# phd3/presto-1

Hardware: AMD Instinct MI355X
Metric: probe_rows_per_sec (higher is better)
Workload: dtype int64+f64

## Files before the change

### presto-1_amd/csrc/basic.hip

```cpp
#include "kernels.h"
#include "device_hash.h"

namespace tgpu {
namespace k {

constexpr int kBlock = 256;
constexpr int kWaves = kBlock / 64;

constexpr int kScanItems = 8;
constexpr int kScanTile = kBlock * kScanItems;

template <typename T> __device__ __forceinline__ T wave_inclusive_scan(T v)
{
    const int lane = threadIdx.x & 63;
#pragma unroll
    for (int d = 1; d < 64; d <<= 1) {
        T t = __shfl_up(v, d, 64);
        if (lane >= d) v += t;
    }
    return v;
}

template <typename T> __device__ __forceinline__ T block_exclusive_scan(T v, T *total, T *lds )
{
    const int lane = threadIdx.x & 63, wave = threadIdx.x >> 6;
    T inc = wave_inclusive_scan(v);
    if (lane == 63) lds[wave] = inc;
    __syncthreads();
    if (threadIdx.x == 0) {
        T run = 0;
#pragma unroll
        for (int w = 0; w < kWaves; w++) { T t = lds[w]; lds[w] = run; run += t; }
        lds[kWaves] = run;
    }
    __syncthreads();
    T prefix = lds[wave] + inc - v;
    *total = lds[kWaves];
    __syncthreads();
    return prefix;
}

__device__ __forceinline__ void scan_load8(const int32_t *__restrict__ in, int64_t idx, int64_t n, bool aligned, int32_t v[kScanItems])
{
    if (aligned && idx + kScanItems <= n) {
        const int4 a = *reinterpret_cast<const int4 *>(in + idx), b = *reinterpret_cast<const int4 *>(in + idx + 4);
        v[0] = a.x; v[1] = a.y; v[2] = a.z; v[3] = a.w; v[4] = b.x; v[5] = b.y; v[6] = b.z; v[7] = b.w;
        return;
    }
#pragma unroll
    for (int i = 0; i < kScanItems; i++) v[i] = idx + i < n ? in[idx + i] : 0;
}

constexpr int kScanMaxBlocks = 2048;

__global__ void __launch_bounds__(kBlock) scan_range_sums_i32(const int32_t *__restrict__ in, int64_t n, int64_t range, int64_t *__restrict__ range_sums)
{
    __shared__ int64_t lds[kWaves + 1];
    const bool aligned = (reinterpret_cast<uintptr_t>(in) & 15) == 0;
    const int64_t a = (int64_t)blockIdx.x * range, z = a + range < n ? a + range : n;
    int64_t s = 0;
    for (int64_t base = a; base < z; base += kScanTile) {
        int32_t v[kScanItems];
        scan_load8(in, base + (int64_t)threadIdx.x * kScanItems, z, aligned, v);
#pragma unroll
        for (int i = 0; i < kScanItems; i++) s += v[i];
    }
    int64_t total;
    block_exclusive_scan<int64_t>(s, &total, lds);
    if (threadIdx.x == 0) range_sums[blockIdx.x] = total;
}

__global__ void __launch_bounds__(kBlock) scan_ranges_i32(const int32_t *__restrict__ in, int32_t *__restrict__ out, int64_t n, int64_t range,
                                                           const int64_t *__restrict__ range_prefix)
{
    __shared__ int64_t lds[kWaves + 1];
    const bool aligned = (reinterpret_cast<uintptr_t>(in) & 15) == 0, out_aligned = (reinterpret_cast<uintptr_t>(out) & 15) == 0;
    const int64_t a = (int64_t)blockIdx.x * range, z = a + range < n ? a + range : n;
    int64_t carry = range_prefix[blockIdx.x];
    for (int64_t base = a; base < z; base += kScanTile) {
        const int64_t idx = base + (int64_t)threadIdx.x * kScanItems;
        int32_t v[kScanItems];
        scan_load8(in, idx, z, aligned, v);
        int64_t s = 0;
#pragma unroll
        for (int i = 0; i < kScanItems; i++) s += v[i];
        int64_t total;
        int64_t prefix = carry + block_exclusive_scan<int64_t>(s, &total, lds);
        int32_t o[kScanItems];
#pragma unroll
        for (int i = 0; i < kScanItems; i++) {
            o[i] = (int32_t)prefix;
            prefix += v[i];
        }
        if (out_aligned && idx + kScanItems <= z) {
            *reinterpret_cast<int4 *>(out + idx) = make_int4(o[0], o[1], o[2], o[3]);
            *reinterpret_cast<int4 *>(out + idx + 4) = make_int4(o[4], o[5], o[6], o[7]);
        } else {
#pragma unroll
            for (int i = 0; i < kScanItems; i++)
                if (idx + i < z) out[idx + i] = o[i];
        }
        carry += total;
    }
}

__global__ void __launch_bounds__(kBlock) scan_small_i64(const int64_t *__restrict__ in, int64_t *__restrict__ out, int64_t n, int64_t *total_out)
{
    __shared__ int64_t lds[kWaves + 1];
    int64_t carry = 0;
    for (int64_t base = 0; base < n; base += kBlock) {
        int64_t idx = base + threadIdx.x;
        int64_t v = idx < n ? in[idx] : 0;
        int64_t total;
        int64_t p = block_exclusive_scan<int64_t>(v, &total, lds);
        if (idx < n) out[idx] = carry + p;
        carry += total;
    }
    if (threadIdx.x == 0 && total_out) *total_out = carry;
}

__global__ void __launch_bounds__(kBlock) scan_one_tile_i32(const int32_t *__restrict__ in, int32_t *__restrict__ out, int64_t n, int64_t *total_out)
{
    __shared__ int64_t lds[kWaves + 1];
    const int64_t base = (int64_t)threadIdx.x * kScanItems;
    int32_t v[kScanItems];
    int64_t s = 0;
#pragma unroll
    for (int i = 0; i < kScanItems; i++) {
        v[i] = base + i < n ? in[base + i] : 0;
        s += v[i];
    }
    int64_t total;
    int64_t prefix = block_exclusive_scan<int64_t>(s, &total, lds);
#pragma unroll
    for (int i = 0; i < kScanItems; i++) {
        if (base + i < n) out[base + i] = (int32_t)prefix;
        prefix += v[i];
    }
    if (threadIdx.x == 0 && total_out) *total_out = total;
}

void exclusive_scan_i32(Context *ctx, const int32_t *in, int32_t *out, int64_t n, int64_t *total_dev)
{
    if (n <= 0) {
        if (total_dev) HIP_CHECK(hipMemsetAsync(total_dev, 0, 8, ctx->stream()));
        return;
    }
    if (n <= kScanTile) {
        scan_one_tile_i32<<<1, kBlock, 0, ctx->stream()>>>(in, out, n, total_dev);
        check_launch("exclusive_scan_i32");
        return;
    }
    const int64_t tiles = ceil_div(n, kScanTile);
    const int64_t tiles_per_range = ceil_div(tiles, (int64_t)kScanMaxBlocks), range = tiles_per_range * kScanTile, ranges = ceil_div(n, range);
    BufferPtr sums = ctx->alloc((size_t)ranges * 8);
    BufferPtr prefix = ctx->alloc((size_t)ranges * 8);
    scan_range_sums_i32<<<(int)ranges, kBlock, 0, ctx->stream()>>>(in, n, range, sums->as<int64_t>());
    scan_small_i64<<<1, kBlock, 0, ctx->stream()>>>(sums->as<int64_t>(), prefix->as<int64_t>(), ranges, total_dev);
    scan_ranges_i32<<<(int)ranges, kBlock, 0, ctx->stream()>>>(in, out, n, range, prefix->as<int64_t>());
    check_launch("exclusive_scan_i32");
}

__global__ void __launch_bounds__(kBlock) hash_rows_kernel(KeyCols keys, int64_t n, int64_t *__restrict__ out)
{
    for (int64_t r = (int64_t)blockIdx.x * kBlock + threadIdx.x; r < n; r += (int64_t)gridDim.x * kBlock) {
        out[r] = tg_hash_row_u(keys, r);
    }
}

void hash_rows(Context *ctx, const KeyCols &keys, int64_t n, int64_t *out)
{
    if (n <= 0) return;
    ProfileScope ps(ctx, "hash_rows");
    hash_rows_kernel<<<grid_for(ctx, n), kBlock, 0, ctx->stream()>>>(keys, n, out);
    check_launch("hash_rows");
}

__global__ void __launch_bounds__(kBlock) any_null_kernel(KeyCols keys, int64_t n, uint8_t *__restrict__ out)
{
    for (int64_t r = (int64_t)blockIdx.x * kBlock + threadIdx.x; r < n; r += (int64_t)gridDim.x * kBlock) {
        uint8_t f = 0;
#pragma unroll
        for (int c = 0; c < TG_MAX_KEY_CHANNELS; c++) {
            if (c >= keys.n) break;
            f |= (keys.c[c].nulls && keys.c[c].nulls[r]) ? 1 : 0;
        }
        out[r] = f;
    }
}

void any_null(Context *ctx, const KeyCols &keys, int64_t n, uint8_t *out)
{
    if (n <= 0) return;
    any_null_kernel<<<grid_for(ctx, n), kBlock, 0, ctx->stream()>>>(keys, n, out);
    check_launch("any_null");
}

template <typename T> __global__ void __launch_bounds__(kBlock) fill_kernel(T *p, T v, int64_t n)
{
    for (int64_t i = (int64_t)blockIdx.x * kBlock + threadIdx.x; i < n; i += (int64_t)gridDim.x * kBlock) p[i] = v;
}
__global__ void __launch_bounds__(kBlock) iota_kernel(int32_t *p, int64_t n)
{
    for (int64_t i = (int64_t)blockIdx.x * kBlock + threadIdx.x; i < n; i += (int64_t)gridDim.x * kBlock) p[i] = (int32_t)i;
}
__global__ void __launch_bounds__(kBlock) widen_kernel(const int32_t *in, int64_t *out, int64_t n)
{
    for (int64_t i = (int64_t)blockIdx.x * kBlock + threadIdx.x; i < n; i += (int64_t)gridDim.x * kBlock) out[i] = in[i];
}

void fill_i32(Context *ctx, int32_t *p, int32_t v, int64_t n)
{
    if (n <= 0) return;
    fill_kernel<int32_t><<<grid_for(ctx, n), kBlock, 0, ctx->stream()>>>(p, v, n);
    check_launch("fill_i32");
}
void fill_u64(Context *ctx, uint64_t *p, uint64_t v, int64_t n)
{
    if (n <= 0) return;
    fill_kernel<uint64_t><<<grid_for(ctx, n), kBlock, 0, ctx->stream()>>>(p, v, n);
    check_launch("fill_u64");
}
void iota_i32(Context *ctx, int32_t *p, int64_t n)
{
    if (n <= 0) return;
    iota_kernel<<<grid_for(ctx, n), kBlock, 0, ctx->stream()>>>(p, n);
    check_launch("iota_i32");
}
void widen_i32_to_i64(Context *ctx, const int32_t *in, int64_t *out, int64_t n)
{
    if (n <= 0) return;
    widen_kernel<<<grid_for(ctx, n), kBlock, 0, ctx->stream()>>>(in, out, n);
    check_launch("widen");
}

__global__ void __launch_bounds__(kBlock) compact_positions_kernel(const int32_t *__restrict__ flags, const int32_t *__restrict__ rank, int64_t n, int32_t *__restrict__ out)
{
    for (int64_t i = (int64_t)blockIdx.x * kBlock + threadIdx.x; i < n; i += (int64_t)gridDim.x * kBlock)
        if (flags[i]) out[rank[i]] = (int32_t)i;
}
void compact_positions(Context *ctx, const int32_t *flags, const int32_t *rank, int64_t n, int32_t *out)
{
    if (n <= 0) return;
    compact_positions_kernel<<<grid_for(ctx, n), kBlock, 0, ctx->stream()>>>(flags, rank, n, out);
}

template <typename T>
__global__ void __launch_bounds__(kBlock) gather_fixed_kernel(const T *__restrict__ src, const uint8_t *__restrict__ src_nulls,
                                                               const int32_t *__restrict__ pos, int64_t n_out,
                                                               T *__restrict__ out, uint8_t *__restrict__ out_nulls)
{
    for (int64_t i = (int64_t)blockIdx.x * kBlock + threadIdx.x; i < n_out; i += (int64_t)gridDim.x * kBlock) {
        int32_t p = pos[i];
        T v = T(0);
        uint8_t isnull = 1;
        if (p >= 0) {
            isnull = src_nulls ? src_nulls[p] : 0;
            v = src[p];
        }
        out[i] = v;
        if (out_nulls) out_nulls[i] = isnull;
    }
}

__global__ void __launch_bounds__(kBlock) gather_len_kernel(const int32_t *__restrict__ offsets, const int32_t *__restrict__ pos,
                                                             int64_t n_out, int32_t *__restrict__ len)
{
    for (int64_t i = (int64_t)blockIdx.x * kBlock + threadIdx.x; i < n_out; i += (int64_t)gridDim.x * kBlock) {
        int32_t p = pos[i];
        len[i] = p >= 0 ? offsets[p + 1] - offsets[p] : 0;
    }
}

__global__ void __launch_bounds__(kBlock) gather_bytes_kernel(const uint8_t *__restrict__ pool, const int32_t *__restrict__ offsets,
                                                               const uint8_t *__restrict__ src_nulls, const int32_t *__restrict__ pos,
                                                               int64_t n_out, const int32_t *__restrict__ out_offsets,
                                                               const int64_t *__restrict__ total, int32_t *__restrict__ out_offsets_end,
                                                               uint8_t *__restrict__ out_pool, uint8_t *__restrict__ out_nulls)
{
    for (int64_t i = (int64_t)blockIdx.x * kBlock + threadIdx.x; i < n_out; i += (int64_t)gridDim.x * kBlock) {
        int32_t p = pos[i];
        uint8_t isnull = 1;
        if (p >= 0) {
            isnull = src_nulls ? src_nulls[p] : 0;
            int32_t a = offsets[p], b = offsets[p + 1], o = out_offsets[i];
            for (int32_t k = a; k < b; k++) out_pool[o + (k - a)] = pool[k];
        }
        if (out_nulls) out_nulls[i] = isnull;
        if (i == n_out - 1) *out_offsets_end = (int32_t)(*total);
    }
}

DeviceColumn gather_column(Context *ctx, const DeviceColumn &src, const int32_t *positions, int64_t n_out, bool negative_is_null)
{
    DeviceColumn out;
    out.type = src.type;
    out.n = n_out;
    const bool need_nulls = src.nulls != nullptr || negative_is_null;
    if (need_nulls) {
        out.nulls_buf = ctx->alloc((size_t)(n_out > 0 ? n_out : 1));
        out.nulls = out.nulls_buf->as<uint8_t>();
    }
// ... 88 lines not shown
```

### presto-1_amd/csrc/join.hip

```cpp
#include "join.h"
#include "kernels.h"
#include "device_hash.h"
#include "device_join.h"

#include <rocprim/rocprim.hpp>

#include <algorithm>
#include <cstdlib>

namespace tgpu {

namespace {

constexpr int kBlock = 256;

using Slot16 = TgSlot16;

__device__ __forceinline__ bool rows_equal_nonnull(const KeyCols &a, int64_t ra, const KeyCols &b, int64_t rb)
{
#pragma unroll
    for (int c = 0; c < TG_MAX_KEY_CHANNELS; c++) {
        if (c >= a.n) break;
        const ColView &x = a.c[c], &y = b.c[c];
        switch (x.type) {
// ... 123 lines not shown
        if (!row_has_null(keys, r)) {
            const int64_t h = hashes[r];
            uint64_t pos = tg_fmix64((uint64_t)h) & mask;
            for (uint64_t iter = 0; iter <= mask; iter++) {
                int *hp = heads + pos * stride;
                int cur = __hip_atomic_load(hp, __ATOMIC_RELAXED, __HIP_MEMORY_SCOPE_AGENT);
                if (cur == -1) {
                    int old = atomicCAS(hp, -1, (int)r);
                    if (old == -1) { slot = (int32_t)pos; break; }
                    cur = old;
                }
                if (tags[cur] == (uint8_t)h && rows_equal_nonnull(keys, cur, keys, r)) {
                    atomicMax(hp, (int)r);
                    slot = (int32_t)pos;
                    dup = true;
                    break;
                }
                pos = (pos + 1) & mask;
                if (iter == mask) atomicExch(&counters[1], 1ull);
            }
        }
        row_slot[r] = slot;
        unsigned long long b = __ballot(dup);
        if (dup && (threadIdx.x & 63) == (__ffsll((long long)b) - 1)) atomicAdd(&counters[0], (unsigned long long)__popcll(b));
    }
}

constexpr long long kUnwrittenKey = (long long)0x8000000000000001ull;
constexpr int kBuildRows = 4;

__device__ __forceinline__ int build_insert_row(const ColView &key, long long k, int r, Slot16 *slots, uint64_t mask, uint64_t pos, long long ks, int head, bool &dup,
                                                unsigned long long *counters)
{
    for (uint64_t iter = 0; iter <= mask; iter++) {
        if (head == -1) {
            const int old = atomicCAS(&slots[pos].head, -1, r);
            if (old == -1) {
                __hip_atomic_store(&slots[pos].key, k, __ATOMIC_RELAXED, __HIP_MEMORY_SCOPE_AGENT);
                return (int)pos;
            }
            head = old;
            ks = __hip_atomic_load(&slots[pos].key, __ATOMIC_RELAXED, __HIP_MEMORY_SCOPE_AGENT);
        }
        const bool same = ks == kUnwrittenKey ? int_key_at(key, head) == k : ks == k;
        if (same) {
            (void)__hip_atomic_fetch_max(&slots[pos].head, r, __ATOMIC_RELAXED, __HIP_MEMORY_SCOPE_AGENT);
            dup = true;
            return (int)pos;
        }
        pos = (pos + 1) & mask;
        const ulonglong2 v = *(const ulonglong2 *)&slots[pos];
        ks = (long long)v.x;
        head = (int)(unsigned int)v.y;
    }
    atomicExch(&counters[1], 1ull);
    return -1;
}

__global__ void __launch_bounds__(kBlock) build_insert_int_kernel(ColView key, int64_t n, Slot16 *slots, uint64_t mask, int32_t *__restrict__ row_slot,
                                                                   unsigned long long *counters, long long *minmax)
{
    long long lo = 0x7fffffffffffffffLL, hi = -0x7fffffffffffffffLL - 1;
    unsigned int my_dups = 0;
    for (int64_t base = (int64_t)blockIdx.x * (kBlock * kBuildRows); base < n; base += (int64_t)gridDim.x * (kBlock * kBuildRows)) {
        long long k[kBuildRows];
        bool live[kBuildRows], claimed[kBuildRows];
        uint64_t pos[kBuildRows];
        ulonglong2 snap[kBuildRows];
        int old[kBuildRows];
#pragma unroll
        for (int u = 0; u < kBuildRows; u++) {
            const int64_t r = base + u * kBlock + threadIdx.x;
            live[u] = r < n && !(key.nulls && key.nulls[r]);
            k[u] = live[u] ? int_key_at(key, r) : 0;
            if (live[u]) {
                lo = k[u] < lo ? k[u] : lo;
                hi = k[u] > hi ? k[u] : hi;
            }
        }
#pragma unroll
        for (int u = 0; u < kBuildRows; u++) {
            pos[u] = tg_slot_of(k[u], mask);
            snap[u] = *(const ulonglong2 *)&slots[live[u] ? pos[u] : 0];
        }
#pragma unroll
        for (int u = 0; u < kBuildRows; u++) {
            claimed[u] = live[u] && (int)(unsigned int)snap[u].y == -1;
            old[u] = 0;
            if (claimed[u]) old[u] = atomicCAS(&slots[pos[u]].head, -1, (int)(base + u * kBlock + threadIdx.x));
        }
#pragma unroll
        for (int u = 0; u < kBuildRows; u++)
            if (claimed[u] && old[u] == -1) __hip_atomic_store(&slots[pos[u]].key, k[u], __ATOMIC_RELAXED, __HIP_MEMORY_SCOPE_AGENT);
#pragma unroll
        for (int u = 0; u < kBuildRows; u++) {
            const int64_t r = base + u * kBlock + threadIdx.x;
            int32_t slot = -1;
            bool dup = false;
            if (claimed[u] && old[u] == -1) slot = (int32_t)pos[u];
            else if (live[u]) {
                long long ks = (long long)snap[u].x;
                int head = (int)(unsigned int)snap[u].y;
                if (claimed[u]) {
                    head = old[u];
                    ks = __hip_atomic_load(&slots[pos[u]].key, __ATOMIC_RELAXED, __HIP_MEMORY_SCOPE_AGENT);
                }
                slot = build_insert_row(key, k[u], (int)r, slots, mask, pos[u], ks, head, dup, counters);
            }
            if (r < n) row_slot[r] = slot;
            my_dups += dup ? 1u : 0u;
        }
    }
    __shared__ unsigned int s_dups[kBlock / 64];
#pragma unroll
    for (int d = 32; d >= 1; d >>= 1) my_dups += __shfl_down(my_dups, d, 64);
    if ((threadIdx.x & 63) == 0) s_dups[threadIdx.x >> 6] = my_dups;
    __syncthreads();
    if (threadIdx.x == 0) {
        unsigned long long total = 0;
#pragma unroll
        for (int w = 0; w < kBlock / 64; w++) total += s_dups[w];
        if (total) atomicAdd(&counters[0], total);
    }
    block_minmax(lo, hi, minmax);
}

__global__ void __launch_bounds__(kBlock) sort_keys_kernel(const int32_t *__restrict__ row_slot, int64_t n, unsigned long long *__restrict__ keys)
{
    for (int64_t r = (int64_t)blockIdx.x * kBlock + threadIdx.x; r < n; r += (int64_t)gridDim.x * kBlock) {
        int32_t s = row_slot[r];
        keys[r] = s < 0 ? ~0ull : (((unsigned long long)(uint32_t)s << 32) | (unsigned long long)(uint32_t)r);
    }
}

__global__ void __launch_bounds__(kBlock) links_kernel(const unsigned long long *__restrict__ sorted, int64_t n, int32_t *__restrict__ links, Slot16 *slots)
{
    for (int64_t i = (int64_t)blockIdx.x * kBlock + threadIdx.x; i < n; i += (int64_t)gridDim.x * kBlock) {
        unsigned long long k = sorted[i];
        if (k == ~0ull) continue;
        int32_t link = -1;
        if (i > 0) {
            unsigned long long p = sorted[i - 1];
            if ((p >> 32) == (k >> 32)) link = (int32_t)(uint32_t)p;
        }
        links[(uint32_t)k] = link;
        if (slots && (i + 1 == n || (sorted[i + 1] >> 32) != (k >> 32))) {
            int64_t first = i;
            while (first > 0 && (sorted[first - 1] >> 32) == (k >> 32)) first--;
            slots[k >> 32].count = (int)(i - first + 1);
        }
    }
}

__global__ void __launch_bounds__(kBlock) key_range_kernel(ColView key, int64_t n, long long *minmax)
{
    long long lo = 0x7fffffffffffffffLL, hi = -0x7fffffffffffffffLL - 1;
    bool descent = false;
    const int64_t stride = (int64_t)gridDim.x * kBlock;
    const int lane = threadIdx.x & 63;
    for (int64_t r0 = (int64_t)blockIdx.x * kBlock + threadIdx.x; r0 < n; r0 += 4 * stride) {
        long long k[4], before[4];
        bool live[4];
#pragma unroll
        for (int u = 0; u < 4; u++) {
            const int64_t r = r0 + u * stride;
            live[u] = r < n;
            const int64_t rc = live[u] ? r : r0;
            live[u] = live[u] && !(key.nulls && key.nulls[rc]);
            k[u] = int_key_at(key, rc);
            before[u] = (lane == 0 && r < n && r > 0) ? int_key_at(key, r - 1) : (-0x7fffffffffffffffLL - 1);
        }
#pragma unroll
        for (int u = 0; u < 4; u++) {
            const int64_t r = r0 + u * stride;
            lo = (live[u] && k[u] < lo) ? k[u] : lo;
            hi = (live[u] && k[u] > hi) ? k[u] : hi;
            const long long up = __shfl_up(k[u], 1, 64);
            const long long pred = lane == 0 ? before[u] : up;
            descent = descent || (r < n && r > 0 && pred >= k[u]);
        }
    }
    block_minmax(lo, hi, minmax);
    if (__any(descent) && (threadIdx.x & 63) == 0) minmax[2] = 1;
}

__global__ void __launch_bounds__(kBlock) build_direct_kernel(ColView key, int64_t n, long long key_min, unsigned long long *bitmap,
                                                               unsigned long long *counters)
{
    const int lane = threadIdx.x & 63;
    unsigned int my_dups = 0;
    for (int64_t base = (int64_t)blockIdx.x * kBlock; base < n; base += (int64_t)gridDim.x * kBlock) {
        const int64_t r = base + threadIdx.x;
        const bool active = r < n && !(key.nulls && key.nulls[r]);
        unsigned long long d = 0;
        if (active) {
            d = (unsigned long long)int_key_at(key, r) - (unsigned long long)key_min;
        }
        const unsigned int word = active ? (unsigned int)(d >> 6) : 0xffffffffu;
        unsigned long long bits = active ? (1ULL << (d & 63)) : 0ULL;
        unsigned int rows = active ? 1u : 0u;
        const unsigned int word_prev = __shfl_up(word, 1, 64);
        const bool head = lane == 0 || word_prev != word;
        const unsigned long long heads = __ballot(head);
        const int run = __popcll(heads & ((2ULL << lane) - 1ULL));
#pragma unroll
        for (int k = 1; k < 64; k <<= 1) {
            const unsigned long long b2 = __shfl_down(bits, k, 64);
            const unsigned int c2 = __shfl_down(rows, k, 64);
            const int run2 = __shfl_down(run, k, 64);
            if (lane + k < 64 && run2 == run) {
                bits |= b2;
                rows += c2;
            }
        }
        if (head && active) {
            const unsigned long long old = atomicOr(&bitmap[word], bits);
            my_dups += (unsigned int)__popcll(old & bits) + (rows - (unsigned int)__popcll(bits));
        }
    }
    __shared__ unsigned int s_dups[kBlock / 64];
#pragma unroll
    for (int d = 32; d >= 1; d >>= 1) my_dups += __shfl_down(my_dups, d, 64);
    if (lane == 0) s_dups[threadIdx.x >> 6] = my_dups;
    __syncthreads();
    if (threadIdx.x == 0) {
        unsigned long long total = 0;
#pragma unroll
        for (int w = 0; w < kBlock / 64; w++) total += s_dups[w];
        if (total) atomicAdd(&counters[0], total);
    }
}

__global__ void __launch_bounds__(kBlock) init_slots_kernel(Slot16 *__restrict__ slots, int64_t capacity)
{
    for (int64_t i = (int64_t)blockIdx.x * kBlock + threadIdx.x; i < capacity; i += (int64_t)gridDim.x * kBlock) {
        Slot16 s;
        s.key = kUnwrittenKey;
        s.head = -1;
        s.count = 1;
        slots[i] = s;
    }
}

__global__ void __launch_bounds__(kBlock) bitmap_popcount_kernel(const unsigned long long *__restrict__ bitmap, int64_t words, int32_t *__restrict__ counts)
{
    for (int64_t i = (int64_t)blockIdx.x * kBlock + threadIdx.x; i < words; i += (int64_t)gridDim.x * kBlock) counts[i] = (int32_t)__popcll(bitmap[i]);
}

__global__ void __launch_bounds__(kBlock) build_rank_kernel(ColView key, int64_t n, long long key_min, const unsigned long long *__restrict__ bitmap,
                                                             const int32_t *__restrict__ rank_base, int32_t *__restrict__ direct)
{
    for (int64_t r = (int64_t)blockIdx.x * kBlock + threadIdx.x; r < n; r += (int64_t)gridDim.x * kBlock) {
        if (key.nulls && key.nulls[r]) continue;
        const unsigned long long d = (unsigned long long)int_key_at(key, r) - (unsigned long long)key_min;
        direct[rank_base[d >> 6] + __popcll(bitmap[d >> 6] & ((1ULL << (d & 63)) - 1ULL))] = (int32_t)r;
    }
}

__global__ void __launch_bounds__(kBlock) bitmap_build_kernel(const int32_t *__restrict__ row_slot, int64_t n, ColView key, long long key_min,
                                                               unsigned long long *bitmap)
{
    for (int64_t r = (int64_t)blockIdx.x * kBlock + threadIdx.x; r < n; r += (int64_t)gridDim.x * kBlock) {
        if (row_slot[r] < 0) continue;
        const unsigned long long d = (unsigned long long)(int_key_at(key, r) - key_min);
        atomicOr(&bitmap[d >> 6], 1ULL << (d & 63));
    }
}

__global__ void __launch_bounds__(kBlock) bloom_build_kernel(const int32_t *__restrict__ row_slot, int64_t n, ColView key, unsigned long long *bloom,
                                                              unsigned long long word_mask)
{
    for (int64_t r = (int64_t)blockIdx.x * kBlock + threadIdx.x; r < n; r += (int64_t)gridDim.x * kBlock) {
        if (row_slot[r] < 0) continue;
        const unsigned long long m = tg_fmix64((unsigned long long)tg_hash_long(int_key_at(key, r)));
        atomicOr(&bloom[tg_bloom_word(m, word_mask)], tg_bloom_mask(m));
    }
}

struct ProbeTable {
    const int *heads;
    const Slot16 *slots;
    const uint8_t *tags;
    const int32_t *links;
    uint64_t mask;
    TgPrefilter pf;
};

template <bool FAST>
__device__ __forceinline__ int find_head(const ProbeTable &t, const KeyCols &build, const KeyCols &probe, int64_t r, int64_t h)
{
    if (FAST) return tg_find_head_int(t.slots, t.mask, t.pf, int_key_at(probe.c[0], r));
    uint64_t pos = tg_fmix64((uint64_t)h) & t.mask;
    for (uint64_t iter = 0; iter <= t.mask; iter++) {
        const int b = t.heads[pos];
        if (b < 0) return -1;
        if (t.tags[b] == (uint8_t)h && rows_equal_nonnull(build, b, probe, r)) return b;
        pos = (pos + 1) & t.mask;
    }
    return -1;
}

template <bool FAST>
__global__ void __launch_bounds__(kBlock) probe_count_kernel(ProbeTable t, KeyCols build, KeyCols probe, const int64_t *__restrict__ hashes, int64_t n,
                                                              int probe_outer, int32_t *__restrict__ heads_out, int32_t *__restrict__ counts)
{
    for (int64_t r = (int64_t)blockIdx.x * kBlock + threadIdx.x; r < n; r += (int64_t)gridDim.x * kBlock) {
        int head = -1, chain = 0;
        if (!row_has_null(probe, r)) {
            if (FAST) head = tg_find_head_int(t.slots, t.mask, t.pf, int_key_at(probe.c[0], r), &chain);
            else head = find_head<FAST>(t, build, probe, r, hashes[r]);
        }
        int32_t c = 0;
        if (head >= 0) {
            c = 1;
            if (t.links) {
                if (FAST && !t.pf.rank_base) c = chain;
                else
                    for (int p = t.links[head]; p >= 0; p = t.links[p]) c++;
            }
        }
        else if (probe_outer) c = 1;
        heads_out[r] = head;
        counts[r] = c;
    }
}

__global__ void __launch_bounds__(kBlock) probe_write_kernel(const int32_t *__restrict__ links, const int32_t *__restrict__ heads, const int32_t *__restrict__ offsets,
                                                              const int32_t *__restrict__ counts, int64_t n, int probe_outer, int32_t *__restrict__ out_probe,
                                                              int32_t *__restrict__ out_build)
{
    for (int64_t r = (int64_t)blockIdx.x * kBlock + threadIdx.x; r < n; r += (int64_t)gridDim.x * kBlock) {
        int head = heads[r];
        int64_t o = offsets[r];
        if (head >= 0) {
            int p = head;
            for (int32_t left = counts[r]; left > 0; left--) {
                out_probe[o] = (int32_t)r;
                out_build[o] = p;
                o++;
                if (left > 1) p = links[p];
            }
        }
        else if (probe_outer) {
            out_probe[o] = (int32_t)r;
            out_build[o] = -1;
        }
    }
}

}

PagesIndexGpu::PagesIndexGpu(Context *ctx, std::vector<int32_t> types) : ctx_(ctx), types_(std::move(types))
{
    cols_.resize(types_.size());
    for (size_t i = 0; i < types_.size(); i++) {
        TG_CHECK_ARG(valid_type(types_[i]), "unknown type");
        cols_[i].type = types_[i];
    }
}

int64_t PagesIndexGpu::estimated_size() const
{
    int64_t s = 0;
    for (auto &c : adopted_) s += c.size_in_bytes();
    for (auto &c : cols_) s += c.cap * type_width(c.type) + (c.nulls ? c.cap : 0) + (c.offsets ? (c.cap + 1) * 4 : 0) + c.pool_cap;
    return s;
}

void PagesIndexGpu::reserve(int64_t rows)
{
    for (auto &c : cols_) {
        if (rows <= c.cap) continue;
// ... 157 lines not shown
{
    std::vector<int32_t> t;
    for (int32_t ch : output_channels_) t.push_back(index_->types()[ch]);
    return t;
}

std::vector<int32_t> LookupSourceGpu::key_types() const
{
    std::vector<int32_t> t;
    for (int32_t ch : key_channels_) t.push_back(index_->types()[ch]);
    return t;
}

int64_t LookupSourceGpu::estimated_size() const
{
    return index_->estimated_size() + (rank_base_ ? (int64_t)((direct_ ? direct_->bytes() : 0) + rank_base_->bytes()) : capacity_ * (int_key_fast_ ? 16 : 4)) + (tags_ ? n_ : 0) + (links_ ? n_ * 4 : 0) +
           (bitmap_ ? (int64_t)bitmap_->bytes() : 0) + (bloom_ ? bloom_words_ * 8 : 0);
}

void LookupSourceGpu::build()
{
    n_ = index_->position_count();
    key_cols_.clear();
    for (int32_t ch : key_channels_) key_cols_.push_back(index_->column(ch));
    int_key_fast_ = key_cols_.size() == 1 && (key_cols_[0].type == TGPU_BIGINT || key_cols_[0].type == TGPU_INTEGER || key_cols_[0].type == TGPU_DATE);
    const double max_load = int_key_fast_ ? 0.5 : 0.75;
    capacity_ = 1024;
    while ((double)capacity_ * max_load < (double)n_) capacity_ <<= 1;
    if (capacity_ > (1ll << 31)) fail(TGPU_ERR_INSUFFICIENT_RESOURCES, "hash table size cannot exceed 2 billion slots");
    link_count_ = 0;
    direct_.reset();
    rank_base_.reset();
    links_.reset();
    tags_.reset();
    bitmap_.reset();
    bloom_.reset();
    heads_.reset();
    slots16_.reset();
    key_min_ = 0;
    key_max_ = -1;
    int *heads = nullptr;
    int stride = 1;
    if (int_key_fast_ && n_ > 0 && getenv("TGPU_DISABLE_DIRECT") == nullptr) {
        std::vector<const DeviceColumn *> kp0;
        for (auto &c : key_cols_) kp0.push_back(&c);
        if (build_direct(key_cols_of(kp0))) return;
    }
    if (int_key_fast_) {
        slots16_ = ctx_->alloc((size_t)capacity_ * 16);
        init_slots_kernel<<<grid_for(ctx_, capacity_), kBlock, 0, ctx_->stream()>>>(slots16_->as<Slot16>(), capacity_);
        check_launch("init_slots");
        heads = &slots16_->as<Slot16>()->head;
        stride = 4;
    }
    else {
        heads_ = ctx_->alloc((size_t)capacity_ * 4);
        k::fill_i32(ctx_, heads_->as<int32_t>(), -1, capacity_);
        heads = heads_->as<int>();
    }
    if (n_ == 0) return;
    std::vector<const DeviceColumn *> kp;
    for (auto &c : key_cols_) kp.push_back(&c);
    const KeyCols keys = key_cols_of(kp);

    BufferPtr row_slot = ctx_->alloc((size_t)n_ * 4);
    BufferPtr counters = ctx_->alloc(32);
    {
        const long long init[4] = {0, 0, 0x7fffffffffffffffLL, -0x7fffffffffffffffLL - 1};
        ctx_->upload(counters->ptr(), init, 32);
    }
    const int g = grid_for(ctx_, n_);
    if (int_key_fast_) {
        ProfileScope ps(ctx_, "join_build_insert");
        build_insert_int_kernel<<<g, kBlock, 0, ctx_->stream()>>>(keys.c[0], n_, slots16_->as<Slot16>(), (uint64_t)capacity_ - 1, row_slot->as<int32_t>(),
                                                                 counters->as<unsigned long long>(), counters->as<long long>() + 2);
        check_launch("build_insert_int");
    }
    else {
        BufferPtr own_hashes;
        const int64_t *hashes;
        DeviceColumn hash_col;
        if (hash_channel_ >= 0) {
            hash_col = index_->column(hash_channel_);
            TG_CHECK_ARG(hash_col.type == TGPU_BIGINT, "hash channel must be BIGINT");
            hashes = (const int64_t *)hash_col.values;
        }
        else {
            own_hashes = ctx_->alloc((size_t)n_ * 8);
            k::hash_rows(ctx_, keys, n_, own_hashes->as<int64_t>());
            hashes = own_hashes->as<int64_t>();
        }
        tags_ = ctx_->alloc((size_t)n_);
        ProfileScope ps(ctx_, "join_build_insert");
        tags_kernel<<<g, kBlock, 0, ctx_->stream()>>>(hashes, n_, tags_->as<uint8_t>());
        build_insert_kernel<<<g, kBlock, 0, ctx_->stream()>>>(keys, hashes, tags_->as<uint8_t>(), n_, heads, stride, (uint64_t)capacity_ - 1,
                                                             row_slot->as<int32_t>(), counters->as<unsigned long long>());
        check_launch("build_insert");
    }
    unsigned long long host_ctr[4];
    ctx_->download(host_ctr, counters->ptr(), 32);
    TG_CHECK_STATE(host_ctr[1] == 0, "join table overflow");
    link_count_ = (int64_t)host_ctr[0];
    if (link_count_ > 0) {
        ProfileScope ps(ctx_, "join_build_links");
        links_ = ctx_->alloc((size_t)n_ * 4);
        k::fill_i32(ctx_, links_->as<int32_t>(), -1, n_);
        BufferPtr keys_in = ctx_->alloc((size_t)n_ * 8), keys_out = ctx_->alloc((size_t)n_ * 8);
        sort_keys_kernel<<<g, kBlock, 0, ctx_->stream()>>>(row_slot->as<int32_t>(), n_, keys_in->as<unsigned long long>());
        size_t temp_bytes = 0;
        HIP_CHECK(rocprim::radix_sort_keys(nullptr, temp_bytes, keys_in->as<unsigned long long>(), keys_out->as<unsigned long long>(), (size_t)n_, 0, 64, ctx_->stream()));
        BufferPtr temp = ctx_->alloc(temp_bytes ? temp_bytes : 1);
        HIP_CHECK(rocprim::radix_sort_keys(temp->ptr(), temp_bytes, keys_in->as<unsigned long long>(), keys_out->as<unsigned long long>(), (size_t)n_, 0, 64, ctx_->stream()));
        links_kernel<<<g, kBlock, 0, ctx_->stream()>>>(keys_out->as<unsigned long long>(), n_, links_->as<int32_t>(), int_key_fast_ ? slots16_->as<Slot16>() : nullptr);
        check_launch("links");
    }
    if (int_key_fast_) {
        ProfileScope ps(ctx_, "join_build_prefilter");
        key_min_ = (long long)host_ctr[2];
        key_max_ = (long long)host_ctr[3];
        const bool has_keys = key_max_ >= key_min_;
        const unsigned long long range = has_keys ? (unsigned long long)key_max_ - (unsigned long long)key_min_ + 1ULL : 0ULL;
        const bool dense = has_keys && range != 0 && range <= (1ULL << 34) && range / 4096ULL <= (unsigned long long)std::max<int64_t>(n_, 1) &&
                           getenv("TGPU_DISABLE_BITMAP") == nullptr;
        if (dense) {
            const int64_t words = (int64_t)((range + 63) / 64);
            bitmap_ = ctx_->alloc_zero((size_t)words * 8);
            bitmap_build_kernel<<<g, kBlock, 0, ctx_->stream()>>>(row_slot->as<int32_t>(), n_, keys.c[0], key_min_, bitmap_->as<unsigned long long>());
            check_launch("bitmap_build");
        }
        else if (has_keys) {
            static const int bits_per_key = getenv("TGPU_BLOOM_BITS_PER_KEY") ? std::max(1, atoi(getenv("TGPU_BLOOM_BITS_PER_KEY"))) : 16;
            int64_t words = 1024;
            while (words * 64 < n_ * bits_per_key) words <<= 1;
            static const int64_t max_bloom_bytes = getenv("TGPU_BLOOM_MAX_BYTES") ? atoll(getenv("TGPU_BLOOM_MAX_BYTES")) : (1ll << 40);
            if (words * 8 <= max_bloom_bytes) {
                bloom_words_ = words;
                bloom_ = ctx_->alloc_zero((size_t)words * 8);
                bloom_build_kernel<<<g, kBlock, 0, ctx_->stream()>>>(row_slot->as<int32_t>(), n_, keys.c[0], bloom_->as<unsigned long long>(), (unsigned long long)words - 1);
                check_launch("bloom_build");
            }
        }
    }
}

bool LookupSourceGpu::build_direct(const KeyCols &keys)
{
    const int g = grid_for(ctx_, n_);
    BufferPtr mm = ctx_->alloc(24);
    const long long init[3] = {0x7fffffffffffffffLL, -0x7fffffffffffffffLL - 1, 0};
    ctx_->upload(mm->ptr(), init, 24);
    long long host_mm[3];
    {
        ProfileScope ps(ctx_, "join_build_range");
        key_range_kernel<<<std::min(g, ctx_->cu_count() * 2), kBlock, 0, ctx_->stream()>>>(keys.c[0], n_, mm->as<long long>());
        check_launch("key_range");
    }
    ctx_->download(host_mm, mm->ptr(), 24);
    if (host_mm[1] < host_mm[0]) return false;
    const bool ascending = host_mm[2] == 0 && keys.c[0].nulls == nullptr && getenv("TGPU_DISABLE_ASCENDING_BUILD") == nullptr;
    const unsigned long long range = (unsigned long long)host_mm[1] - (unsigned long long)host_mm[0] + 1ULL;
    if (range == 0 || range > (1ULL << 31) || range / 64ULL > (unsigned long long)n_) return false;
    const int64_t words = (int64_t)((range + 63) / 64);
    BufferPtr bitmap = ctx_->alloc_zero((size_t)words * 8);
    BufferPtr direct = ascending ? nullptr : ctx_->alloc((size_t)n_ * 4);
    BufferPtr rank_base = ctx_->alloc((size_t)words * 4);
    BufferPtr counters = ctx_->alloc_zero(16);
    {
        ProfileScope ps(ctx_, "join_build_insert");
        build_direct_kernel<<<g, kBlock, 0, ctx_->stream()>>>(keys.c[0], n_, host_mm[0], bitmap->as<unsigned long long>(), counters->as<unsigned long long>());
        check_launch("build_direct");
    }
    if (!ascending && ctx_->read_scalar(counters->as<unsigned long long>()) != 0) return false;
    key_min_ = host_mm[0];
    key_max_ = host_mm[1];
    bitmap_ = bitmap;
    direct_ = direct;
    rank_base_ = rank_base;
    direct_key_ = keys.c[0];
    rank_pending_ = true;
    if (!output_channels_.empty()) ensure_rank();
    return true;
}

void LookupSourceGpu::ensure_rank() const
{
    if (!rank_base_) return;
    std::lock_guard<std::mutex> lk(visited_mu_);
    if (!rank_pending_) return;
    const int64_t range = (int64_t)((unsigned long long)key_max_ - (unsigned long long)key_min_ + 1ULL);
    const int64_t words = (range + 63) / 64;
    ProfileScope ps(ctx_, "join_build_rank");
    BufferPtr counts = ctx_->alloc((size_t)words * 4), total = ctx_->alloc(8);
    bitmap_popcount_kernel<<<grid_for(ctx_, words), kBlock, 0, ctx_->stream()>>>(bitmap_->as<unsigned long long>(), words, counts->as<int32_t>());
    check_launch("bitmap_popcount");
    k::exclusive_scan_i32(ctx_, counts->as<int32_t>(), rank_base_->as<int32_t>(), words, total->as<int64_t>());
    if (direct_) {
        build_rank_kernel<<<grid_for(ctx_, n_), kBlock, 0, ctx_->stream()>>>(direct_key_, n_, key_min_, bitmap_->as<unsigned long long>(), rank_base_->as<int32_t>(),
                                                                            direct_->as<int32_t>());
        check_launch("build_rank");
    }
    rank_pending_ = false;
}

bool LookupSourceGpu::int_table(IntTableView &v) const
{
    if (!int_key_fast_ || (!slots16_ && !rank_base_)) return false;
    v.slots = slots16_ ? slots16_->ptr() : nullptr;
    v.direct = direct_ ? direct_->as<int32_t>() : nullptr;
    v.rank_base = rank_base_ ? rank_base_->as<int32_t>() : nullptr;
    v.mask = (uint64_t)capacity_ - 1;
    v.bloom = bloom_ ? bloom_->as<unsigned long long>() : nullptr;
    v.bloom_word_mask = bloom_ ? (unsigned long long)bloom_words_ - 1 : 0;
    v.bitmap = bitmap_ ? bitmap_->as<unsigned long long>() : nullptr;
    v.key_min = key_min_;
    v.key_max = key_max_;
    v.links = links_ ? links_->as<int32_t>() : nullptr;
    v.key_type = key_cols_.empty() ? index_->types()[(size_t)key_channels_[0]] : key_cols_[0].type;
    return true;
}

void LookupSourceGpu::probe(const std::vector<const DeviceColumn *> &probe_keys, const int64_t *probe_hashes, int64_t n, bool probe_outer,
                            BufferPtr &out_probe_idx, BufferPtr &out_build_idx, int64_t &out_count)
{
    TG_CHECK_ARG(probe_keys.size() == key_channels_.size(), "probe key channel count differs from the build side's");
    for (size_t i = 0; i < probe_keys.size(); i++) {
        const int32_t bt = index_->types()[key_channels_[i]];
        const bool int_like = (bt == TGPU_BIGINT || bt == TGPU_INTEGER || bt == TGPU_DATE);
        TG_CHECK_ARG(probe_keys[i]->type == bt || (int_key_fast_ && int_like && probe_keys[i]->type == bt), "probe key type differs from the build key type");
    }
    out_count = 0;
    if (n <= 0) {
        out_probe_idx = ctx_->alloc(4);
        out_build_idx = ctx_->alloc(4);
        return;
    }
    ensure_rank();
    const KeyCols probe = key_cols_of(probe_keys);
    std::vector<const DeviceColumn *> kp;
    for (auto &c : key_cols_) kp.push_back(&c);
    const KeyCols build = key_cols_.empty() ? KeyCols{} : key_cols_of(kp);
    BufferPtr own_hashes;
    if (!probe_hashes && !int_key_fast_) {
        own_hashes = ctx_->alloc((size_t)n * 8);
        k::hash_rows(ctx_, probe, n, own_hashes->as<int64_t>());
        probe_hashes = own_hashes->as<int64_t>();
    }
    ProbeTable t{};
    t.heads = heads_ ? heads_->as<int>() : nullptr;
    t.slots = slots16_ ? slots16_->as<Slot16>() : nullptr;
    t.tags = tags_ ? tags_->as<uint8_t>() : nullptr;
    t.links = links_ ? links_->as<int32_t>() : nullptr;
    t.mask = (uint64_t)capacity_ - 1;
    t.pf.bitmap = bitmap_ ? bitmap_->as<unsigned long long>() : nullptr;
    t.pf.key_min = key_min_;
    t.pf.key_max = key_max_;
    t.pf.bloom = bloom_ ? bloom_->as<unsigned long long>() : nullptr;
    t.pf.bloom_word_mask = bloom_ ? (unsigned long long)bloom_words_ - 1 : 0;
    t.pf.direct = direct_ ? direct_->as<int>() : nullptr;
    t.pf.rank_base = rank_base_ ? rank_base_->as<int>() : nullptr;
    BufferPtr heads = ctx_->alloc((size_t)n * 4), counts = ctx_->alloc((size_t)n * 4), offsets = ctx_->alloc((size_t)n * 4), total = ctx_->alloc(8);
    const int g = grid_for(ctx_, n);
    {
        ProfileScope ps(ctx_, "join_probe_count");
        if (int_key_fast_)
            probe_count_kernel<true><<<g, kBlock, 0, ctx_->stream()>>>(t, build, probe, probe_hashes, n, probe_outer ? 1 : 0, heads->as<int32_t>(), counts->as<int32_t>());
        else
            probe_count_kernel<false><<<g, kBlock, 0, ctx_->stream()>>>(t, build, probe, probe_hashes, n, probe_outer ? 1 : 0, heads->as<int32_t>(), counts->as<int32_t>());
        check_launch("probe_count");
    }
    {
        ProfileScope ps(ctx_, "join_probe_scan");
        k::exclusive_scan_i32(ctx_, counts->as<int32_t>(), offsets->as<int32_t>(), n, total->as<int64_t>());
    }
    out_count = ctx_->read_scalar(total->as<int64_t>());
    if (out_count > 0x7fffffffLL) fail(TGPU_ERR_INSUFFICIENT_RESOURCES, "join output of one probe page cannot exceed 2 billion rows");
    out_probe_idx = ctx_->alloc((size_t)(out_count > 0 ? out_count : 1) * 4);
    out_build_idx = ctx_->alloc((size_t)(out_count > 0 ? out_count : 1) * 4);
    if (out_count > 0) {
        ProfileScope ps(ctx_, "join_probe_write");
        probe_write_kernel<<<g, kBlock, 0, ctx_->stream()>>>(t.links, heads->as<int32_t>(), offsets->as<int32_t>(), counts->as<int32_t>(), n, probe_outer ? 1 : 0,
                                                            out_probe_idx->as<int32_t>(), out_build_idx->as<int32_t>());
        check_launch("probe_write");
    }
}

DeviceColumn LookupSourceGpu::gather_index_channel(int channel, const int32_t *build_positions, int64_t n) const
{
    TG_CHECK_ARG(channel >= 0 && channel < (int)index_->types().size(), "build channel out of range");
    return k::gather_column(ctx_, index_->column(channel), build_positions, n, false);
}

DeviceColumn LookupSourceGpu::build_column(int out_idx) const { return index_->column(output_channels_[out_idx]); }

DeviceColumn LookupSourceGpu::gather_build(int out_idx, const int32_t *build_positions, int64_t n, bool negative_is_null) const
{
    DeviceColumn src = index_->column(output_channels_[out_idx]);
    if (src.type != TGPU_VARCHAR && src.values == nullptr) {
        BufferPtr dummy = ctx_->alloc(8);
        src.values_buf = dummy;
        src.values = dummy->ptr();
    }
    if (src.type == TGPU_VARCHAR && src.offsets == nullptr) {
        BufferPtr off = ctx_->alloc_zero(8), pool = ctx_->alloc(8);
        src.offsets_buf = off;
        src.offsets = off->as<int32_t>();
        src.values_buf = pool;
        src.values = pool->ptr();
    }
    return k::gather_column(ctx_, src, build_positions, n, negative_is_null);
}


namespace {
__global__ void __launch_bounds__(kBlock) mark_visited_kernel(const int32_t *__restrict__ positions, int64_t n, uint8_t *__restrict__ visited)
{
    for (int64_t i = (int64_t)blockIdx.x * kBlock + threadIdx.x; i < n; i += (int64_t)gridDim.x * kBlock) {
        const int32_t p = positions[i];
        if (p >= 0) visited[p] = 1;
    }
}
__global__ void __launch_bounds__(kBlock) unvisited_flags_kernel(const uint8_t *__restrict__ visited, int64_t n, int32_t *__restrict__ flags)
{
    for (int64_t i = (int64_t)blockIdx.x * kBlock + threadIdx.x; i < n; i += (int64_t)gridDim.x * kBlock) flags[i] = (visited && visited[i]) ? 0 : 1;
}
}

void LookupSourceGpu::mark_visited(const int32_t *build_positions, int64_t n)
{
    if (n <= 0 || n_ <= 0) return;
    {
        std::lock_guard<std::mutex> lk(visited_mu_);
        if (!visited_) visited_ = ctx_->alloc_zero((size_t)n_);
// ... 21 lines not shown
```

Baseline: 93.16 billion.

## Vectorize key range scan, derive rank from heads, add mid-size scan

The key-range kernel gains a 128-bit paired-load path for non-null aligned bigint keys, a template unroll factor, and fewer blocks per CU by default. For ascending keys, the direct-build kernel writes each bitmap word's rank base from the first row index in that word. This skips the popcount-plus-scan rank pass and the duplicate counter. A single-block 1024-thread scan kernel with vectorized loads and stores is added for mid-size inputs. These changes mainly cut build-side cost, which may matter little for a probe-rows metric. The ascending rank shortcut depends on the rank matching the row index, which holds only when there are no duplicates or gaps.

```diff
diff --git a/presto-1_amd/csrc/basic.hip b/presto-1_amd/csrc/basic.hip
--- a/presto-1_amd/csrc/basic.hip
+++ b/presto-1_amd/csrc/basic.hip
@@ -140,6 +140,52 @@
     if (threadIdx.x == 0 && total_out) *total_out = total;
 }
 
+constexpr int kScanMidBlock = 1024, kScanMidItems = 16, kScanMid = kScanMidBlock * kScanMidItems;
+
+__global__ void __launch_bounds__(kScanMidBlock) scan_mid_i32(const int32_t *__restrict__ in, int32_t *__restrict__ out, int64_t n, int64_t *total_out)
+{
+    __shared__ int64_t wave_total[kScanMidBlock / 64];
+    const int lane = threadIdx.x & 63, wave = threadIdx.x >> 6;
+    const bool aligned = (reinterpret_cast<uintptr_t>(in) & 15) == 0, out_aligned = (reinterpret_cast<uintptr_t>(out) & 15) == 0;
+    const int64_t base = (int64_t)threadIdx.x * kScanMidItems;
+    int32_t v[kScanMidItems];
+#pragma unroll
+    for (int q = 0; q < kScanMidItems; q += 4) {
+        if (aligned && base + q + 4 <= n) {
+            const int4 a = *reinterpret_cast<const int4 *>(in + base + q);
+            v[q] = a.x; v[q + 1] = a.y; v[q + 2] = a.z; v[q + 3] = a.w;
+        } else {
+#pragma unroll
+            for (int i = q; i < q + 4; i++) v[i] = base + i < n ? in[base + i] : 0;
+        }
+    }
+    int64_t s = 0;
+#pragma unroll
+    for (int i = 0; i < kScanMidItems; i++) s += v[i];
+    const int64_t inc = wave_inclusive_scan<int64_t>(s);
+    if (lane == 63) wave_total[wave] = inc;
+    __syncthreads();
+    const int64_t t = lane < kScanMidBlock / 64 ? wave_total[lane] : 0;
+    const int64_t tinc = wave_inclusive_scan<int64_t>(t);
+    int64_t prefix = __shfl(tinc - t, wave, 64) + inc - s;
+    int32_t o[kScanMidItems];
+#pragma unroll
+    for (int i = 0; i < kScanMidItems; i++) {
+        o[i] = (int32_t)prefix;
+        prefix += v[i];
+    }
+#pragma unroll
+    for (int q = 0; q < kScanMidItems; q += 4) {
+        if (out_aligned && base + q + 4 <= n) *reinterpret_cast<int4 *>(out + base + q) = make_int4(o[q], o[q + 1], o[q + 2], o[q + 3]);
+        else {
+#pragma unroll
+            for (int i = q; i < q + 4; i++)
+                if (base + i < n) out[base + i] = o[i];
+        }
+    }
+    if (threadIdx.x == kScanMidBlock - 1 && total_out) *total_out = tinc;
+}
+
 void exclusive_scan_i32(Context *ctx, const int32_t *in, int32_t *out, int64_t n, int64_t *total_dev)
 {
     if (n <= 0) {
@@ -148,6 +194,11 @@
     }
     if (n <= kScanTile) {
         scan_one_tile_i32<<<1, kBlock, 0, ctx->stream()>>>(in, out, n, total_dev);
+        check_launch("exclusive_scan_i32");
+        return;
+    }
+    if (n <= kScanMid) {
+        scan_mid_i32<<<1, kScanMidBlock, 0, ctx->stream()>>>(in, out, n, total_dev);
         check_launch("exclusive_scan_i32");
         return;
     }
diff --git a/presto-1_amd/csrc/join.hip b/presto-1_amd/csrc/join.hip
--- a/presto-1_amd/csrc/join.hip
+++ b/presto-1_amd/csrc/join.hip
@@ -299,13 +299,45 @@
     }
 }
 
+constexpr int kRangeLoads = 8, kRangeBlocksPerCu = 1;
+
+template <int U>
 __global__ void __launch_bounds__(kBlock) key_range_kernel(ColView key, int64_t n, long long *minmax)
 {
-    long long lo = 0x7fffffffffffffffLL, hi = -0x7fffffffffffffffLL - 1;
+    constexpr long long kMin = -0x7fffffffffffffffLL - 1;
+    long long lo = 0x7fffffffffffffffLL, hi = kMin;
     bool descent = false;
     const int64_t stride = (int64_t)gridDim.x * kBlock;
     const int lane = threadIdx.x & 63;
-    for (int64_t r0 = (int64_t)blockIdx.x * kBlock + threadIdx.x; r0 < n; r0 += 4 * stride) {
+    const bool wide = key.type == TGPU_BIGINT && key.nulls == nullptr && (reinterpret_cast<uintptr_t>(key.values) & 15) == 0;
+    const int64_t pairs = wide ? n / 2 : 0;
+    if (wide) {
+        const longlong2 *__restrict__ kv = (const longlong2 *)key.values;
+        const long long *__restrict__ ks = (const long long *)key.values;
+        for (int64_t p0 = (int64_t)blockIdx.x * kBlock + threadIdx.x; p0 < pairs; p0 += U * stride) {
+            longlong2 k[U];
+            long long before[U];
+#pragma unroll
+            for (int u = 0; u < U; u++) {
+                const int64_t p = p0 + u * stride, pc = p < pairs ? p : p0;
+                k[u] = kv[pc];
+                const int64_t first = pc - lane;
+                before[u] = ks[first > 0 ? 2 * first - 1 : 0];
+            }
+#pragma unroll
+            for (int u = 0; u < U; u++) {
+                const int64_t p = p0 + u * stride;
+                const bool live = p < pairs;
+                const long long a = k[u].x < k[u].y ? k[u].x : k[u].y, z = k[u].x < k[u].y ? k[u].y : k[u].x;
+                lo = (live && a < lo) ? a : lo;
+                hi = (live && z > hi) ? z : hi;
+                const long long up = __shfl_up(k[u].y, 1, 64);
+                const long long pred = lane == 0 ? before[u] : up;
+                descent |= live & ((k[u].x >= k[u].y) | ((p > 0) & (pred >= k[u].x)));
+            }
+        }
+    }
+    for (int64_t r0 = 2 * pairs + (int64_t)blockIdx.x * kBlock + threadIdx.x; r0 < n; r0 += 4 * stride) {
         long long k[4], before[4];
         bool live[4];
 #pragma unroll
@@ -315,7 +347,7 @@
             const int64_t rc = live[u] ? r : r0;
             live[u] = live[u] && !(key.nulls && key.nulls[rc]);
             k[u] = int_key_at(key, rc);
-            before[u] = (lane == 0 && r < n && r > 0) ? int_key_at(key, r - 1) : (-0x7fffffffffffffffLL - 1);
+            before[u] = (lane == 0 && r < n && r > 0) ? int_key_at(key, r - 1) : kMin;
         }
 #pragma unroll
         for (int u = 0; u < 4; u++) {
@@ -331,19 +363,22 @@
     if (__any(descent) && (threadIdx.x & 63) == 0) minmax[2] = 1;
 }
 
+template <bool ASC>
 __global__ void __launch_bounds__(kBlock) build_direct_kernel(ColView key, int64_t n, long long key_min, unsigned long long *bitmap,
-                                                               unsigned long long *counters)
+                                                               unsigned long long *counters, int32_t *__restrict__ rank_base)
 {
     const int lane = threadIdx.x & 63;
     unsigned int my_dups = 0;
     for (int64_t base = (int64_t)blockIdx.x * kBlock; base < n; base += (int64_t)gridDim.x * kBlock) {
         const int64_t r = base + threadIdx.x;
-        const bool active = r < n && !(key.nulls && key.nulls[r]);
+        const bool active = r < n && (ASC || !(key.nulls && key.nulls[r]));
         unsigned long long d = 0;
         if (active) {
             d = (unsigned long long)int_key_at(key, r) - (unsigned long long)key_min;
         }
         const unsigned int word = active ? (unsigned int)(d >> 6) : 0xffffffffu;
+        unsigned int word_before = 0xffffffffu;
+        if (ASC && lane == 0 && active && r > 0) word_before = (unsigned int)(((unsigned long long)int_key_at(key, r - 1) - (unsigned long long)key_min) >> 6);
         unsigned long long bits = active ? (1ULL << (d & 63)) : 0ULL;
         unsigned int rows = active ? 1u : 0u;
         const unsigned int word_prev = __shfl_up(word, 1, 64);
@@ -361,10 +396,17 @@
             }
         }
         if (head && active) {
-            const unsigned long long old = atomicOr(&bitmap[word], bits);
-            my_dups += (unsigned int)__popcll(old & bits) + (rows - (unsigned int)__popcll(bits));
-        }
-    }
+            if (ASC) {
+                atomicOr(&bitmap[word], bits);
+                if (lane != 0 || word_before != word) rank_base[word] = (int32_t)r;
+            }
+            else {
+                const unsigned long long old = atomicOr(&bitmap[word], bits);
+                my_dups += (unsigned int)__popcll(old & bits) + (rows - (unsigned int)__popcll(bits));
+            }
+        }
+    }
+    if (ASC) return;
     __shared__ unsigned int s_dups[kBlock / 64];
 #pragma unroll
     for (int d = 32; d >= 1; d >>= 1) my_dups += __shfl_down(my_dups, d, 64);
@@ -828,7 +870,14 @@
     long long host_mm[3];
     {
         ProfileScope ps(ctx_, "join_build_range");
-        key_range_kernel<<<std::min(g, ctx_->cu_count() * 2), kBlock, 0, ctx_->stream()>>>(keys.c[0], n_, mm->as<long long>());
+        const char *loads_env = getenv("TGPU_KEY_RANGE_LOADS"), *blocks_env = getenv("TGPU_KEY_RANGE_BLOCKS");
+        const int loads = loads_env ? atoi(loads_env) : kRangeLoads;
+        const int grid = std::min(g, ctx_->cu_count() * (blocks_env ? std::min(std::max(atoi(blocks_env), 1), 8) : kRangeBlocksPerCu));
+        long long *out = mm->as<long long>();
+        if (loads == 2) key_range_kernel<2><<<grid, kBlock, 0, ctx_->stream()>>>(keys.c[0], n_, out);
+        else if (loads == 4) key_range_kernel<4><<<grid, kBlock, 0, ctx_->stream()>>>(keys.c[0], n_, out);
+        else if (loads == 16) key_range_kernel<16><<<grid, kBlock, 0, ctx_->stream()>>>(keys.c[0], n_, out);
+        else key_range_kernel<kRangeLoads><<<grid, kBlock, 0, ctx_->stream()>>>(keys.c[0], n_, out);
         check_launch("key_range");
     }
     ctx_->download(host_mm, mm->ptr(), 24);
@@ -840,20 +889,29 @@
     BufferPtr bitmap = ctx_->alloc_zero((size_t)words * 8);
     BufferPtr direct = ascending ? nullptr : ctx_->alloc((size_t)n_ * 4);
     BufferPtr rank_base = ctx_->alloc((size_t)words * 4);
-    BufferPtr counters = ctx_->alloc_zero(16);
-    {
+    const char *from_heads_env = getenv("TGPU_DIRECT_RANK_FROM_HEADS");
+    const bool rank_from_heads = ascending && !(from_heads_env && atoi(from_heads_env) == 0);
+    if (rank_from_heads) {
         ProfileScope ps(ctx_, "join_build_insert");
-        build_direct_kernel<<<g, kBlock, 0, ctx_->stream()>>>(keys.c[0], n_, host_mm[0], bitmap->as<unsigned long long>(), counters->as<unsigned long long>());
+        build_direct_kernel<true><<<g, kBlock, 0, ctx_->stream()>>>(keys.c[0], n_, host_mm[0], bitmap->as<unsigned long long>(), nullptr, rank_base->as<int32_t>());
         check_launch("build_direct");
     }
-    if (!ascending && ctx_->read_scalar(counters->as<unsigned long long>()) != 0) return false;
+    else {
+        BufferPtr counters = ctx_->alloc_zero(16);
+        {
+            ProfileScope ps(ctx_, "join_build_insert");
+            build_direct_kernel<false><<<g, kBlock, 0, ctx_->stream()>>>(keys.c[0], n_, host_mm[0], bitmap->as<unsigned long long>(), counters->as<unsigned long long>(), nullptr);
+            check_launch("build_direct");
+        }
+        if (!ascending && ctx_->read_scalar(counters->as<unsigned long long>()) != 0) return false;
+    }
     key_min_ = host_mm[0];
     key_max_ = host_mm[1];
     bitmap_ = bitmap;
     direct_ = direct;
     rank_base_ = rank_base;
     direct_key_ = keys.c[0];
-    rank_pending_ = true;
+    rank_pending_ = !rank_from_heads;
     if (!output_channels_.empty()) ensure_rank();
     return true;
 }
```

Measured after the change: 96.03 billion (median of 6 runs). 1.03x the previous value.
